# vanilladucky/sde_sampler_lrds

Measured on AMD Instinct MI355X. Metric: particle-steps/sec (batch*n_steps/wall) + log-Z abs-err vs ref, higher is better.
Workload: dtype f32

## Files before the change

sde_sampler_lrds_amd/csrc/prep_kernels.hip:

```cpp
#include "sim_device.hpp"
#include "prep_kernels.hpp"

__global__ void __launch_bounds__(256) k_weight_scales(PackArgs a) {
  __shared__ float red[256];
  float* sc = a.out + sd_off_scales(a.NT);
  {
    const int l = blockIdx.x;
    const float* W = l == 0 ? a.w_in : (l == 1 ? a.w_h1 : (l == 2 ? a.w_h2 : a.w_out));
    const int n = (l == 0 || l == 3) ? SD_H * a.d : SD_H * SD_H;
    float m = 0.0f;
    for (int i = threadIdx.x; i < n; i += 256) {
      const float v = __builtin_fabsf(W[i]);
      m = (v <= 3.0e38f) ? fmaxf(m, v) : m;
    }
    red[threadIdx.x] = m;
    __syncthreads();
    for (int s = 128; s > 0; s >>= 1) {
      if (threadIdx.x < s) red[threadIdx.x] = fmaxf(red[threadIdx.x], red[threadIdx.x + s]);
      __syncthreads();
    }
    if (threadIdx.x == 0) {
      const float mx = red[0];
      int e = 0;
      if (mx > 0.0f && (mx < 9.765625e-4f || mx >= 16384.0f)) {
// ... 78 lines not shown
    float acc = 0.0f;
    for (int i = 0; i < n_in; ++i) acc = __builtin_fmaf(W[i], in[i], acc);
    acc += a.te.b[l][j];
    hbuf[cur][j] = gelu_exact(acc);
    __syncthreads();
    in = hbuf[cur];
    n_in = 64;
    cur ^= 1;
  }
  if (j < a.te.dim_out) {
    const float* W = a.te.w_out + static_cast<size_t>(j) * 64;
    float acc = 0.0f;
    for (int i = 0; i < 64; ++i) acc = __builtin_fmaf(W[i], in[i], acc);
    acc += a.te.b_out[j];
    if (a.clip > 0.0f) acc = clampf(acc, a.clip);
    a.out[static_cast<size_t>(k) * a.te.dim_out + j] = acc;
  }
}

__global__ void __launch_bounds__(128) k_same_var(const float* vars, int K, int d, float* same_var) {
  int differ = 0;
  for (int i = threadIdx.x; i < K * d; i += 128) differ |= vars[i] != vars[i % d];
  differ = __syncthreads_or(differ);
  if (threadIdx.x == 0) same_var[0] = differ ? 0.0f : 1.0f;
}

__global__ void __launch_bounds__(128) k_ref_tables(RefTabArgs a) {
  __shared__ float red[128];
  const int k = blockIdx.x / a.K, c = blockIdx.x % a.K;
  const float S = a.coef[static_cast<size_t>(k) * SDENG_NCOEF + 9];
  const float VA = a.coef[static_cast<size_t>(k) * SDENG_NCOEF + 10];
  const float S2 = a.coef[static_cast<size_t>(k) * SDENG_NCOEF + 11];
  const bool centred = a.centred && a.K == SD_KREG && a.same_var[0] != 0.0f;
  float* tm = a.tab + (static_cast<size_t>(k) * a.K + c) * 2 * a.dpad;
  float* tv = tm + a.dpad;
  float ls = 0.0f, quad = 0.0f;
  for (int f = threadIdx.x; f < a.dpad; f += 128) {
    float mean = 0.0f, iv = 0.0f, cen = 0.0f;
    if (f < a.d) {
      mean = S * a.means[static_cast<size_t>(c) * a.d + f];
      const float var = VA + S2 * a.vars[static_cast<size_t>(c) * a.d + f];
      iv = 1.0f / var;
      ls += logf(var);
      if (centred) {
        float sum = 0.0f;
        for (int j = 0; j < SD_KREG; ++j) sum += a.means[static_cast<size_t>(j) * a.d + f];
        cen = S * (sum * (1.0f / SD_KREG));
      }
    }
    if (centred) {
      const float dm = mean - cen;
      quad = __builtin_fmaf(dm * dm, iv, quad);
      tm[f] = dm * iv;
      tv[f] = c == 0 ? iv : (c == 1 ? cen : 0.0f);
    } else {
      tm[f] = mean;
      tv[f] = iv;
    }
  }
  red[threadIdx.x] = ls;
  __syncthreads();
  for (int s = 64; s > 0; s >>= 1) {
    if (threadIdx.x < s) red[threadIdx.x] += red[threadIdx.x + s];
    __syncthreads();
  }
  const float ls_sum = red[0];
  __syncthreads();
  red[threadIdx.x] = quad;
  __syncthreads();
  for (int s = 64; s > 0; s >>= 1) {
    if (threadIdx.x < s) red[threadIdx.x] += red[threadIdx.x + s];
    __syncthreads();
  }
  if (threadIdx.x == 0) {
    float wsum = 0.0f;
    for (int i = 0; i < a.K; ++i) wsum += a.weights ? a.weights[i] : 1.0f;
    const float w = (a.weights ? a.weights[c] : 1.0f) / wsum;
    float* cs = a.consts + (static_cast<size_t>(k) * a.K + c) * 2;
    cs[0] = 0.5f * ls_sum;
    cs[1] = centred ? logf(w) - 0.5f * red[0] : logf(w);
  }
}

__global__ void __launch_bounds__(256) k_ref_full_tables(RefFullArgs a) {
  __shared__ float invd[128];
  __shared__ float red[256];
  const int k = blockIdx.x / a.K, c = blockIdx.x % a.K;
  const float S = a.coef ? a.coef[static_cast<size_t>(k) * SDENG_NCOEF + 9] : 1.0f;
  const float VA = a.coef ? a.coef[static_cast<size_t>(k) * SDENG_NCOEF + 10] : 0.0f;
  const float S2 = a.coef ? a.coef[static_cast<size_t>(k) * SDENG_NCOEF + 11] : 1.0f;
  const int KB = sd_kb(a.NT);
  const int img_floats = a.NT * KB * 512;
  float ls = 0.0f;
  for (int j = threadIdx.x; j < 128; j += 256) {
    float iv = 0.0f;
    if (j < a.d) {
      const float var = VA + S2 * a.eigvals[static_cast<size_t>(c) * a.d + j];
      iv = 1.0f / var;
      ls += logf(var);
    }
    invd[j] = iv;
  }
  red[threadIdx.x] = ls;
  __syncthreads();
  for (int s = 128; s > 0; s >>= 1) {
    if (threadIdx.x < s) red[threadIdx.x] += red[threadIdx.x + s];
    __syncthreads();
// ... 799 lines not shown
```

sde_sampler_lrds_amd/csrc/prep_kernels.hpp:

```cpp
#pragma once
#include "sim_common.hpp"
#include "../../include/sdeng.h"

#define SD_LOGZ_MAX_BLOCKS 1024

struct PackArgs {
  int NT, d;
  const float *w_in, *b_in, *w_h1, *b_h1, *w_h2, *b_h2, *w_out, *b_out;
  float* out;
  int transpose;
  const float* scales;
};

struct TimeEmbedArgs {
  sdeng_time_embed te;
  const float* coef;
  int col;
  int t_direct;
  float t_value;
  float clip;
  float* out;
};

struct RefTabArgs {
  int K, d, dpad;
  const float* coef;
  const float *means, *vars, *weights;
  float* tab;
  float* consts;
  float* same_var;
  int centred;
};

struct RefFullArgs {
  int K, d, dpad, NT;
  const float* coef;
  const float *means, *eigvals, *eigvecs, *weights;
  float* images;
  float* means_out;
  float* consts;
};

struct RefMMArgs {
  int K, d, dpad, NT, kt;
  const float* coef;
  const float *means, *vars, *weights;
  float* images;
  float* centre;
  float* consts;
  float* same_var;
};

struct DistTabArgs {
  int K, d, dpad;
  const float *loc, *scale, *weights;
  float* tab;
  float* consts;
};

struct DistEvalArgs {
  DistDev ds;
  int B, d, dpad;
  const float* x;
  float* logp_out;
  float* score_out;
};

struct MovesArgs {
  DistEvalArgs prior, target;
  int B, d, K, keep_from, ula;
  float target_acc;
  const float* t;
  float *x, *lp, *grad, *step;
  const float *z, *u;
  unsigned seed_lo, seed_hi;
  long long chain0;
  float* samples;
  float* acc_sum;
  float* acc_last;
};
int sd_launch_moves(const MovesArgs& a, hipStream_t s);

struct TerminalArgs {
  DistDev ref, target;
// ... 18 lines not shown
```

sde_sampler_lrds_amd/csrc/sdeng_api.hip:

```cpp
#include <hip/hip_runtime.h>

#include <algorithm>
#include <cmath>
#include <cstdarg>
#include <cstdio>
#include <cstring>
#include <cstdlib>

#include "../../include/sdeng.h"
#include "prep_kernels.hpp"
#include "sim_kernel.hpp"
#include "cmcd_kernel.hpp"
#include "grad_kernel.hpp"
#include "cmcd_adjoint_kernel.hpp"
#include "metric_kernels.hpp"

int sd_launch_logreg_images(const float* X, const float* y, int n, int dw, int NT, float* image, float* y_pad, hipStream_t s);
int sd_launch_pack_square(const float* P, const float* loc, int d, int NT, float* out, float* loc_pad, hipStream_t s);

static thread_local char g_err[512] = "";
static int fail(int code, const char* fmt, ...) {
  va_list ap;
  va_start(ap, fmt);
  vsnprintf(g_err, sizeof(g_err), fmt, ap);
// ... 500 lines not shown
  SD_TRY(launch_timed(d, p.k, &c, s));
  if (eubo) return terminal(d, dpad, prior, prior, true, false, d->x_out, d->rnd_out, s);
  return terminal(d, dpad, target, target, false, true, d->x_out, d->rnd_out, s);
}

static int run_euler(const SimPlan& p, const sdeng_desc* d, float* ws, SimArgs& a, hipStream_t s) {
  SD_TRY(build_dist(d->target, d->d, 16 * p.DT, ws + p.L.target, a.target, s));
  a.clip_score = d->net.clip_score;
  return launch_timed(d, p.k, &a, s);
}

static int prepare_ref(const SimPlan& p, const sdeng_desc* d, float* ws, SimArgs& a, hipStream_t s) {
  const Layout& L = p.L;
  const int DT = p.DT, dpad = 16 * DT, K = ref_components(d), rf = p.rf;
  if (rf == RF_NONE) return 0;
  a.ref_k = K;
  a.ref_tab = ws + L.ref_tab; a.ref_consts = ws + L.ref_consts;
  a.ref_c1 = half_d_log_2pi(d->d);
  if (rf == RF_GMM_FULL) {
    if (d->N > 0) {
      RefFullArgs r;
      r.K = K; r.d = d->d; r.dpad = dpad; r.NT = DT; r.coef = p.in_slot ? nullptr : d->coef;
      r.means = d->ref.means_init; r.eigvals = d->ref.vars_init; r.eigvecs = d->ref.eigvecs; r.weights = d->ref.weights;
      r.images = ws + L.ref_tab; r.means_out = ws + L.ref_mean; r.consts = ws + L.ref_consts;
      SD_HIP(sd_launch_ref_full_tables(r, d->N, s));
    }
    a.ref_mean = ws + L.ref_mean;
    const int piece = (DT > 4 ? DT / 2 : DT) * sd_kb(DT) * 512;
    a.ref_share = (piece / 256 + SD_WAVES - 1) / SD_WAVES;
    return 0;
  }
  if (rf == RF_GMM_MM) {
    const int kt = (K + 15) / 16;
    if (d->N > 0) {
      RefMMArgs r;
      r.K = K; r.d = d->d; r.dpad = dpad; r.NT = DT; r.kt = kt; r.coef = d->coef;
      r.means = d->ref.means_init; r.vars = d->ref.vars_init; r.weights = d->ref.weights;
      r.images = ws + L.ref_tab; r.centre = ws + L.ref_mean; r.consts = ws + L.ref_consts;
      r.same_var = ws + L.ref_consts + static_cast<size_t>(d->N) * 64;
      SD_HIP(sd_launch_ref_mm_tables(r, d->N, s));
    }
    a.ref_kc = kt;
    a.ref_mean = ws + L.ref_mean;
    a.ref_share = (mm_piece(K, DT) / 256 + SD_WAVES - 1) / SD_WAVES;
    return 0;
  }
  if (d->N > 0) {
    RefTabArgs r;
    r.K = K; r.d = d->d; r.dpad = dpad; r.coef = d->coef;
    r.means = d->ref.means_init; r.vars = d->ref.vars_init; r.weights = rf != RF_GAUSS ? d->ref.weights : nullptr;
    r.tab = ws + L.ref_tab; r.consts = ws + L.ref_consts;
    r.same_var = ws + L.ref_consts + static_cast<size_t>(d->N) * K * 2;
    r.centred = (rf == RF_GMM && p.k.fam != SD_FAM_SPLIT) ? 1 : 0;
    SD_HIP(sd_launch_ref_tables(r, d->N, s));
  }
  a.ref_same_var = ws + L.ref_consts + static_cast<size_t>(d->N) * K * 2;
  if (rf == RF_GMM_BIG) {
    static const bool allow = [] { const char* e = getenv("SDENG_REF_SHARE"); return !(e && e[0] == '0'); }();
    const int cap = std::min(share_room(DT), sd_share_buf_floats(SD_SHARE_MAX)) / 256 * 256;
    const int kc_max = cap / (2 * dpad);
    if (allow && kc_max >= 1) {
      const int nch = (K + kc_max - 1) / kc_max;
      const int kc = (K + nch - 1) / nch;
      const int chunks = (kc * 2 * dpad + 255) / 256;
      a.ref_share = (chunks + SD_WAVES - 1) / SD_WAVES;
      a.ref_kc = kc;
    }
  }
  return 0;
}

static int run_sim(const SimPlan& p, const sdeng_desc* d, float* ws, SimArgs& a, hipStream_t s) {
  const Layout& L = p.L;
  const int DT = p.DT, dpad = 16 * DT;
  SD_TRY(prepare_net(d, L, ws, DT, a, s, d->N, false, 0.0f));
  SD_TRY(prepare_ref(p, d, ws, a, s));
  DistDev target, ref_dist, prior;
  SD_TRY(build_dist(d->target, d->d, dpad, ws + L.target, target, s));
  SD_TRY(build_dist(d->ref_dist, d->d, dpad, ws + L.ref_dist, ref_dist, s));
  SD_TRY(build_dist(d->prior, d->d, dpad, ws + L.prior, prior, s));
  a.target = target;
  a.prior = prior;
  const bool eubo = d->form == SDENG_FORM_EUBO;
  const bool tr = d->flags & SDENG_FLAG_TERM_REF, tt = d->flags & SDENG_FLAG_TERM_TARGET;
  if ((d->flags & SDENG_FLAG_INIT_LOGP) && !eubo) {
    SD_TRY(dist_eval(prior, d->B, d->d, dpad, d->x_in, ws + L.rnd_init, nullptr, s));
    a.rnd_init = ws + L.rnd_init;
  }
  if (eubo && (tr || tt)) {
    SD_HIP(hipMemsetAsync(ws + L.rnd_init, 0, sizeof(float) * d->B, s));
    SD_TRY(terminal(d, dpad, ref_dist, target, tr, tt, d->x_in, ws + L.rnd_init, s));
    a.rnd_init = ws + L.rnd_init;
  }
  if (p.sc == SC_LOGREG) {
    float* unused;
    SD_TRY(prepare_logreg(d, L, ws, DT, a, s, &unused));
  }
  SD_TRY(launch_timed(d, p.k, &a, s));
  if (!eubo && (tr || tt)) SD_TRY(terminal(d, dpad, ref_dist, target, tr, tt, d->x_out, d->rnd_out, s));
  if (eubo && (d->flags & SDENG_FLAG_INIT_LOGP)) SD_TRY(terminal(d, dpad, prior, prior, true, false, d->x_out, d->rnd_out, s));
  return 0;
}

extern "C" int sdeng_simulate(const sdeng_desc* desc, void* stream) {
  hipStream_t s = static_cast<hipStream_t>(stream);
  SimPlan p;
// ... 146 lines not shown
static int check_adjoint(const sdeng_desc* d, bool ext_score) {
  if (!d) return fail(SDENG_E_INVALID, "null descriptor");
  SD_TRY(check_abi(d));
  if (d->d < 1 || d->d > 128 || d->N < 1 || d->B < 1 || !d->coef) return fail(SDENG_E_INVALID, "bad sizes (1 <= d <= 128, N, B >= 1) or null coef");
  if (d->form != SDENG_FORM_LIN && d->form != SDENG_FORM_EM) return fail(SDENG_E_UNSUPPORTED, "kl_adjoint: forward forms LIN / EM (form %d)", d->form);
  if (d->net.ctrl_kind != SDENG_CTRL_CLIPPED &&
      !(score_like(d->net.ctrl_kind) && (ext_score || d->target.kind == SDENG_DIST_GMM_DIAG || d->target.kind == SDENG_DIST_PHI4)))
    return fail(SDENG_E_UNSUPPORTED, "kl_adjoint: ClippedCtrl, or Score / Lerp / CancelDrift control on a diagonal mixture / phi^4 target (ctrl_kind %d, "
                                     "target kind %d)", d->net.ctrl_kind, d->target.kind);
  SD_TRY(check_lerp_prior(d));
  if (d->target.kind == SDENG_DIST_CHECKERBOARD || d->prior.kind == SDENG_DIST_CHECKERBOARD)
    return fail(SDENG_E_UNSUPPORTED, "kl_adjoint: no adjoint for a checkerboard target (KL training takes the per-step path)");
  if (d->ref.kind != SDENG_REF_NONE && d->ref.kind != SDENG_REF_GAUSS_DIAG && d->ref.kind != SDENG_REF_GMM_DIAG)
    return fail(SDENG_E_UNSUPPORTED, "kl_adjoint: no reference, or a diagonal Gaussian / mixture reference (ref.kind %d)", d->ref.kind);
  if (d->ref.kind != SDENG_REF_NONE && ((d->ref.kind == SDENG_REF_GMM_DIAG && d->ref.k < 1) || !d->ref.means_init || !d->ref.vars_init))
    return fail(SDENG_E_INVALID, "reference: null means/vars or k < 1");
  if (static_cast<long long>(d->N) * d->B * d->d >= (1ll << 31)) return fail(SDENG_E_UNSUPPORTED, "N * B * d >= 2^31");
  return check_net(d->net);
}
extern "C" size_t sdeng_kl_adjoint_workspace_bytes(const sdeng_desc* d) {
  if (!d || d->d < 1 || d->d > 128 || d->N < 1) return 0;
  return adjoint_layout(d, tiles_exact(d->d)).total * sizeof(float);
}
extern "C" int sdeng_kl_adjoint(const sdeng_desc* d, const sdeng_adjoint* adj, void* stream) {
  hipStream_t s = static_cast<hipStream_t>(stream);
  SD_TRY(check_adjoint(d, adj && adj->score));
  if (!adj || !adj->xs || !adj->w || !adj->lam_in || !adj->a0 || !adj->a1 || !adj->a2 || !adj->d0 || !adj->d1 || !adj->d2 || !adj->dout)
    return fail(SDENG_E_INVALID, "kl_adjoint: null states / weights / lambda_N / per-row outputs");
  const bool ito = d->flags & SDENG_FLAG_ITO;
  if (ito && !adj->noise) return fail(SDENG_E_INVALID, "kl_adjoint: FLAG_ITO needs the normals of the trajectory");
  const bool score = d->net.ctrl_kind != SDENG_CTRL_CLIPPED;
  if (score && !adj->dst) return fail(SDENG_E_INVALID, "kl_adjoint: a score control needs the dst output");
  if (score && !adj->score) SD_TRY(check_dist(d->target, d->d));
  const int has_score = !score ? ADJ_NONE : adj->score ? ADJ_EXT : (d->target.kind == SDENG_DIST_PHI4 ? ADJ_PHI4 : ADJ_GMM);
  const int DT = tiles_exact(d->d), dpad = 16 * DT;
  KernelKey k;
  SD_TRY(select_kernel(k, SD_FAM_ADJ, DT, has_score));
  const AdjLayout A = adjoint_layout(d, DT);
  const size_t need = A.total * sizeof(float);
  if (!d->workspace || d->workspace_bytes < need) return fail(SDENG_E_WORKSPACE, "workspace %zu bytes, need %zu", d->workspace_bytes, need);
  float* ws = static_cast<float*>(d->workspace);
  AdjArgs a;
  memset(&a, 0, sizeof(a));
  SD_TRY(pack_net(d, DT, ws, ws + A.v.wt, s));
  SD_TRY(embed_times(d, d->N, false, 0.0f, ws + A.v.temb, ws + A.stheta, &a.stheta, s));
  if (d->ref.kind != SDENG_REF_NONE) {
    const int K = ref_components(d);
    RefTabArgs r;
    r.K = K; r.d = d->d; r.dpad = dpad; r.coef = d->coef;
    r.means = d->ref.means_init; r.vars = d->ref.vars_init; r.weights = d->ref.kind == SDENG_REF_GMM_DIAG ? d->ref.weights : nullptr;
    r.tab = ws + A.tab; r.consts = ws + A.consts;
    r.same_var = ws + A.consts + static_cast<size_t>(d->N) * K * 2;
    r.centred = 0;
    SD_HIP(sd_launch_ref_tables(r, d->N, s));
    a.ref_tab = ws + A.tab; a.ref_consts = ws + A.consts; a.ref_k = K;
    a.ref_c1 = half_d_log_2pi(d->d);
  }
  a.has_score = has_score;
  if (score) {
    a.score_ext = adj->score;
    if (!adj->score) SD_TRY(build_dist(d->target, d->d, dpad, ws + A.target, a.target, s));
    a.scale_score = d->net.scale_score; a.clip_score = d->net.clip_score;
    a.ctrl_kind = d->net.ctrl_kind;
    a.prior_loc = d->prior.p0; a.prior_scale = d->net.ctrl_kind == SDENG_CTRL_LERP ? d->prior.p1 : 1.0f;
    a.score_detached = adj->detach_score ? 1 : 0;
    a.dst = adj->dst;
  }
  VjpArgs& v = a.v;
  v.M = d->N * d->B; v.B = d->B; v.d = d->d; v.N = d->N;
  v.x = adj->xs; v.cot = nullptr; v.wpack = ws; v.wpack_t = ws + A.v.wt; v.temb = ws + A.v.temb;
  v.clip_model = d->net.clip_model;
  v.a0 = adj->a0; v.a1 = adj->a1; v.a2 = adj->a2; v.d0 = adj->d0; v.d1 = adj->d1; v.d2 = adj->d2; v.dout = adj->dout;
  v.trash = ws + A.v.trash;
  a.coef = d->coef; a.noise = ito ? adj->noise : nullptr; a.w = adj->w; a.lam_in = adj->lam_in; a.lam_out = adj->lam_out;
  a.lin = d->form == SDENG_FORM_LIN ? 1 : 0;
  a.ntiles_b = (d->B + 15) / 16;
  SD_HIP(k.fn(&a, s));
  return 0;
}

struct CmcdAdjLayout {
  VjpLayout v;
  size_t stheta, target, prior, total;
};
static CmcdAdjLayout cmcd_adjoint_layout(const sdeng_desc* d, int DT) {
  CmcdAdjLayout A;
  A.v = vjp_layout(DT, d->N + 1);
  size_t o = A.v.total;
  A.stheta = o; o += align64(static_cast<size_t>(d->N) + 1);
  A.target = o; o += dist_floats(d->target, 16 * DT);
  A.prior = o; o += dist_floats(d->prior, 16 * DT);
  A.total = o;
  return A;
}
static int check_cmcd_adjoint(const sdeng_desc* d, bool ext_score) {
  if (!d) return fail(SDENG_E_INVALID, "null descriptor");
  SD_TRY(check_abi(d));
  if (d->d > 128) return fail(SDENG_E_UNSUPPORTED, "cmcd_kl_adjoint: d <= 128 (got %d)", d->d);
  if (d->d < 1 || d->N < 1 || d->B < 1 || !d->coef) return fail(SDENG_E_INVALID, "bad sizes (1 <= d, N, B >= 1) or null coef");
  if (d->net.ctrl_kind != SDENG_CTRL_CLIPPED && d->net.ctrl_kind != SDENG_CTRL_SCORE)
    return fail(SDENG_E_UNSUPPORTED, "cmcd_kl_adjoint: ClippedCtrl or ScoreCtrl (ctrl_kind %d)", d->net.ctrl_kind);
  if (d->prior.kind == SDENG_DIST_GAUSS_FULL)
    return fail(SDENG_E_UNSUPPORTED, "cmcd_kl_adjoint: no adjoint for a full-covariance prior (KL training takes the per-step path)");
  if (d->prior.kind != SDENG_DIST_ISO_GAUSS && d->prior.kind != SDENG_DIST_GAUSS_DIAG)
    return fail(SDENG_E_UNSUPPORTED, "cmcd_kl_adjoint: prior must be ISO_GAUSS or GAUSS_DIAG (kind %d)", d->prior.kind);
  switch (d->target.kind) {
// ... 204 lines not shown
```

sde_sampler_lrds_amd/csrc/sim_device.hpp:

```cpp
#pragma once
#include "sim_common.hpp"
#include "../../include/sdeng.h"

#define SD_INLINE __device__ __forceinline__

SD_INLINE float group_sum(float v) {
  v += __shfl_xor(v, 16, 64);
  v += __shfl_xor(v, 32, 64);
  return v;
}
SD_INLINE float exp_nonpos(float v) { return __builtin_amdgcn_exp2f(v * 1.4426950408889634f); }
SD_INLINE float rcp_fast(float v) { return __builtin_amdgcn_rcpf(v); }

SD_INLINE float clampf(float v, float m) {
  v = (v < -m) ? -m : v;
  v = (v > m) ? m : v;
  return v;
}

SD_INLINE void clamp_tile_rare(f32x4& v, float m) {
  bool out_of_range = false;
#pragma unroll
  for (int r = 0; r < 4; ++r) out_of_range |= !(__builtin_fabsf(v[r]) <= m);
  if (__builtin_amdgcn_ballot_w64(out_of_range) != 0) {
// ... 602 lines not shown
#pragma unroll
  for (int r = 0; r < 4; ++r) acc[r] = (acc[r] - x[t][r]) * iv[r];
  return acc;
}

template <int NT>
SD_INLINE void gmm_resp_centred(const f32x4 (&x)[NT], const float* __restrict__ tab, const float* __restrict__ consts, int g,
                                float (&p)[SD_KREG]) {
  constexpr int dpad = 16 * NT;
  float lp[SD_KREG];
#pragma unroll
  for (int k = 0; k < SD_KREG; ++k) lp[k] = 0.0f;
#pragma unroll
  for (int t = 0; t < NT; ++t) {
    const f32x4 y = x[t] - load_tile4(tab + 3 * dpad, t, g);
#pragma unroll
    for (int k = 0; k < SD_KREG; ++k) {
      const f32x4 ak = load_tile4(tab + static_cast<size_t>(k) * 2 * dpad, t, g);
#pragma unroll
      for (int r = 0; r < 4; ++r) lp[k] = __builtin_fmaf(y[r], ak[r], lp[k]);
    }
  }
  float mx = -INFINITY;
#pragma unroll
  for (int k = 0; k < SD_KREG; ++k) {
    lp[k] = consts[2 * k + 1] + group_sum(lp[k]);
    mx = fmaxf(mx, lp[k]);
  }
  float den = 0.0f;
#pragma unroll
  for (int k = 0; k < SD_KREG; ++k) {
    p[k] = exp_nonpos(lp[k] - mx);
    den += p[k];
  }
  const float inv = rcp_fast(den);
#pragma unroll
  for (int k = 0; k < SD_KREG; ++k) p[k] *= inv;
}
template <int NT>
SD_INLINE f32x4 gmm_score_tile_centred(const f32x4 (&x)[NT], const float* __restrict__ tab, int g, const float (&p)[SD_KREG], int t) {
  constexpr int dpad = 16 * NT;
  f32x4 acc = {0.0f, 0.0f, 0.0f, 0.0f};
#pragma unroll
  for (int k = 0; k < SD_KREG; ++k) {
    const f32x4 ak = load_tile4(tab + static_cast<size_t>(k) * 2 * dpad, t, g);
#pragma unroll
    for (int r = 0; r < 4; ++r) acc[r] = __builtin_fmaf(p[k], ak[r], acc[r]);
  }
  const f32x4 iv = load_tile4(tab + dpad, t, g), c = load_tile4(tab + 3 * dpad, t, g);
#pragma unroll
  for (int r = 0; r < 4; ++r) acc[r] = __builtin_fmaf(c[r] - x[t][r], iv[r], acc[r]);
  return acc;
}

template <int NT>
SD_INLINE f32x4 gauss_score_tile(const f32x4 (&x)[NT], const float* __restrict__ tab, int g, int t) {
  constexpr int dpad = 16 * NT;
  const f32x4 m = load_tile4(tab, t, g);
  const f32x4 iv = load_tile4(tab + dpad, t, g);
  f32x4 out;
#pragma unroll
  for (int r = 0; r < 4; ++r) out[r] = -((x[t][r] - m[r]) * iv[r]);
  return out;
}

SD_INLINE f32x4 rings_score(const f32x4& x, const DistDev& ds, int g) {
  const float n = __builtin_sqrtf(x[0] * x[0] + x[1] * x[1]) + 1e-7f;
  const float var = ds.p0 * ds.p0;
  float wsum = 0.0f;
  for (int k = 0; k < ds.k; ++k) wsum += ds.aux1[k];
  const float cn = 0.5f * 1.8378770664093453f + 0.5f * logf(var);
  float lp[8], mx = -INFINITY;
#pragma unroll
  for (int k = 0; k < 8; ++k) {
    lp[k] = -INFINITY;
    if (k < ds.k) {
      const float dl = n - ds.aux0[k];
      lp[k] = logf(ds.aux1[k] / wsum) + ((-0.5f * ((dl * dl) / var)) - cn);
      mx = fmaxf(mx, lp[k]);
    }
  }
  float den = 0.0f, acc = 0.0f;
#pragma unroll
  for (int k = 0; k < 8; ++k) {
    if (k < ds.k) {
      const float e = expf(lp[k] - mx);
      den += e;
      acc += e * ((n - ds.aux0[k]) / var);
    }
  }
  const float sr = -(acc / den);
  const float f = (sr / n) - (1.0f / (n * n));
  return g == 0 ? f32x4{x[0] * f, x[1] * f, 0.0f, 0.0f} : f32x4{0.0f, 0.0f, 0.0f, 0.0f};
}

template <int NT>
SD_INLINE void phi4_edges(const f32x4 (&x)[NT], int t, int g, int lane, float& l_edge, float& r_edge) {
  const int up = (lane + 48) & 63, dn = (lane + 16) & 63;
  const float l_same = __shfl(x[t][3], up, 64);
  const float r_same = __shfl(x[t][0], dn, 64);
  float l_prev = 0.0f, r_next = 0.0f;
  if (t > 0) l_prev = __shfl(x[t > 0 ? t - 1 : 0][3], up, 64);
  if (t < NT - 1) r_next = __shfl(x[t < NT - 1 ? t + 1 : t][0], dn, 64);
  l_edge = (g == 0) ? l_prev : l_same;
  r_edge = (g == 3) ? r_next : r_same;
}
// ... 136 lines not shown
```

sde_sampler_lrds_amd/csrc/sim_kernel.hpp:

```cpp
#pragma once
#include <type_traits>

#include "sim_device.hpp"

enum { RF_NONE = 0, RF_GAUSS = 1, RF_GMM = 2, RF_GMM_BIG = 3, RF_GMM_FULL = 4, RF_GMM_MM = 5 };
enum { SC_NONE = 0, SC_GMM = 1, SC_PHI4 = 2, SC_LOGREG = 3, SC_REFSLOT = 4 };

template <int KIND, bool CLIP>
SD_INLINE float ctrl_score_term(const SimArgs& a, float sv, float xv, float st, float score_gain, float lerp_w, bool in_range,
                                float inv_prior_var) {
  constexpr bool lerp = KIND == SDENG_CTRL_LERP;
  if constexpr (lerp) {
    const float ps = (a.prior.p0 - xv) * inv_prior_var;
    const float df = sv - ps;
    sv = (lerp_w < 0.5f) ? ps + lerp_w * df : sv - df * (1.0f - lerp_w);
  }
  if constexpr (CLIP) sv = clampf(sv, a.clip_score);
  float v = a.scale_score * sv;
  v = v * st;
  if constexpr (lerp) v = in_range ? score_gain * v : 0.0f;
  if constexpr (KIND == SDENG_CTRL_CANCEL_DRIFT) v = in_range ? lerp_w * xv + score_gain * v : 0.0f;
  return v;
}
template <int KIND, bool CLIP>
// ... 78 lines not shown
    if constexpr (SC == SC_LOGREG) {
      const int ni = a.lr.in_lds ? sd_lr_floats(NT, a.lr.n_rows) / 4 : 0;
      for (int i = tid; i < ni; i += THREADS) dst[n4 + i] = reinterpret_cast<const f32x4*>(a.lr.image)[i];
    }
  }
  __syncthreads();
#ifdef SD_STAGGER
  if constexpr (REF != RF_GMM_BIG && REF != RF_GMM_FULL && REF != RF_GMM_MM)
    if (wave >= W / 2)
      for (int i = 0; i < SD_STAGGER; ++i) __builtin_amdgcn_s_sleep(127);
#endif
#ifdef SD_DBG_PRIO_HI47
  if (wave >= 4) __builtin_amdgcn_s_setprio(3);
#endif
#ifdef SD_DBG_ONLY47
  if (wave < 4) return;
#endif
#ifdef SD_DBG_ONLY03
  if (wave >= 4) return;
#endif
  static_assert(SC != SC_LOGREG || (REF == RF_NONE && NT <= 4), "in-loop logistic-regression score: no reference, d <= 64");
  static_assert(SC != SC_REFSLOT || (REF == RF_GMM_FULL && FORM != SDENG_FORM_EUBO), "full-covariance target score: lives in the reference slot, forward forms");
  constexpr bool has_ref = REF != RF_NONE && SC != SC_REFSLOT;
  const float* bias = a.wpack + sd_off_bias(NT);
  const NetScale ns = load_net_scale(bias, NT);
#ifdef SD_NO_RANGE_GUARD
  const bool scaled_net = false;
#else
  const bool scaled_net = ns.any_hidden();
#endif
  const float inv_out_plain = ns.inv_out;
#ifdef SD_DBG_NODMA
  constexpr bool ref_lds = false;
#else
  constexpr bool ref_lds = (REF == RF_GAUSS || REF == RF_GMM);
#endif
  float* my_tab = lds + sd_lds_weight_floats(NT) + wave * SD_REFTAB_FLOATS;
  const int tab_floats = a.ref_k * 2 * dpad;
  const int share = (REF == RF_GMM_BIG || REF == RF_GMM_FULL || REF == RF_GMM_MM) ? __builtin_amdgcn_readfirstlane(a.ref_share) : 0;
  float* sh_tab = lds + sd_lds_weight_floats(NT);
  const int sh_floats = sd_share_buf_floats(share);
  constexpr int FULL_PP = NT > 4 ? 2 : 1, FULL_TO = NT / FULL_PP, FULL_PIECE = FULL_TO * ((NT + 1) / 2) * 512;
  static_assert(REF != RF_GMM_FULL || NT % FULL_PP == 0, "pieces hold whole output tiles");
  const int p = lane & 15, g = lane >> 4;
  constexpr bool lin = FORM == SDENG_FORM_LIN;
  constexpr bool eubo = FORM == SDENG_FORM_EUBO;
  static_assert(!eubo || (SC == SC_NONE) != (REF == RF_NONE), "EUBO kernels: reference-SDE losses with a ClippedCtrl, or DIS (no reference)");
  const bool full_d = a.d == dpad;
  float* trash = a.trash + tid * 4;
  bool same_var = false;
  if constexpr (REF == RF_GMM) same_var = a.N > 0 && a.ref_same_var[0] != 0.0f;
  const bool kfull = REF == RF_GMM && a.ref_k == SD_KREG;
  const bool kfast = kfull && same_var;

  for (int tile = blockIdx.x + gridDim.x * wave; (share ? tile - static_cast<int>(gridDim.x) * wave : tile) < a.ntiles;
       tile += gridDim.x * W) {
    const uint32_t row = static_cast<uint32_t>(tile) * 16u + p;
    const bool live = row < static_cast<uint32_t>(a.B);
    const uint32_t pidx = static_cast<uint32_t>(a.particle0 + row);
    f32x4 x[NT];
    load_rows<NT>(a.x_in, row, a.d, live, g, x);
    float rnd = 0.0f;
    if (a.rnd_init) rnd = (live ? a.rnd_init[row] : 0.0f);
    if constexpr (PAR) {
      if (a.xs_out) store_rows<NT>(a.xs_out, trash, row, a.d, live, g, x);
    }
    if constexpr (ref_lds) {
      if (a.N > 0) dma_table_to_lds(a.ref_tab, my_tab, tab_floats, lane);
    }
    if constexpr (REF == RF_GMM_BIG) {
      if (share) {
        __syncthreads();
        if (a.N > 0) dma_table_shared(a.ref_tab, sh_tab, min(a.ref_kc, a.ref_k) * 2 * dpad, share, wave, lane);
      }
    }
    if constexpr (REF == RF_GMM_MM) {
      __syncthreads();
      if (a.N > 0) dma_table_shared(a.ref_tab, sh_tab, a.ref_kc * ((NT + 1) / 2) * 512, share, wave, lane);
    }
    if constexpr (REF == RF_GMM_FULL) {
      __syncthreads();
      if (a.N > 0) dma_table_shared(a.ref_tab, sh_tab, FULL_PIECE, share, wave, lane);
    }

    for (int k = 0; k < a.N; ++k) {
      const float* cf = a.coef + static_cast<size_t>(k) * SDENG_NCOEF;
      const float c1 = cf[1], c2 = cf[2], c3 = cf[3], c4 = cf[4], c5 = cf[5], c6 = cf[6];
      const float score_gain = cf[7], lerp_w = cf[8];
      const float e1 = __builtin_fmaf(c4, c1, 1.0f), e2 = c4 * c2, e3 = c4 * c3, e4 = c2 * c5;
      int d_dyn = a.d;
      asm volatile("" : "+s"(d_dyn));

      auto noise_tile = [&](int t) -> f32x4 {
        if (PAR && a.noise_in) return load_quad(a.noise_in + static_cast<size_t>(k) * a.B * a.d, row, d_dyn, live, t, g);
        f32x4 z = philox_normal4(pidx, static_cast<uint32_t>(k), static_cast<uint32_t>(4 * t + g), 0u, a.seed_lo, a.seed_hi);
        if constexpr (SC == SC_PHI4) {
          if (!full_d) {
#pragma unroll
            for (int r = 0; r < 4; ++r) z[r] = feat_live<NT>(t, r, 4 * g, d_dyn) ? z[r] : 0.0f;
          }
        }
        return z;
      };
      if constexpr (eubo) {
#pragma unroll
        for (int t = 0; t < NT; ++t) {
          const f32x4 z = noise_tile(t);
#pragma unroll
          for (int r = 0; r < 4; ++r) x[t][r] = x[t][r] * c1 + c3 * z[r];
        }
      }

      f32x4 hid[SD_HT];
      __builtin_amdgcn_s_setprio(2);
      constexpr bool has_twin = REF != RF_GMM_MM && REF != RF_GMM_FULL && SC != SC_LOGREG;
      if constexpr (has_twin) mlp_hidden<NT>(x, hid, lds, bias, a.temb + static_cast<size_t>(k) * SD_H, lane);
      else mlp_hidden_scaled<NT>(x, hid, lds, bias, a.temb + static_cast<size_t>(k) * SD_H, lane, ns);
      __builtin_amdgcn_s_setprio(1);
      HidSplit hs = split_hidden(hid);
      bool safe_net = false;
      float hid_rs = 1.0f;

      f32x4 ts[(SC != SC_NONE && SC != SC_REFSLOT) ? NT : 1];
      if constexpr (SC == SC_GMM) {
        if (NT == 1 && a.target.kind == SDENG_DIST_RINGS) ts[0] = rings_score(x[0], a.target, g);
        else gmm_score<NT>(x, a.target.tab, a.target.consts, 4, a.target.k, a.target.p0, g, ts);
      }
      if constexpr (SC == SC_PHI4) {
        int lane_p = lane;
        if constexpr (NT == 8) asm volatile("" : "+v"(lane_p));
        phi4_score<NT>(x, a.target, d_dyn, g, lane_p, ts);
      }
      if constexpr (SC == SC_LOGREG) {
        asm volatile("" ::: "memory");
        f16x8 xh[(NT + 1) / 2], xl[(NT + 1) / 2];
        split_tiles<NT>(x, xh, xl);
        if (a.lr.in_lds) logreg_score<NT>(x, xh, xl, a.lr, d_dyn, lds + sd_lds_weight_floats(NT), lane, ts);
        else logreg_score<NT>(x, xh, xl, a.lr, d_dyn, a.lr.image, lane, ts);
      }
      const float* rtab = ref_lds ? my_tab : a.ref_tab + static_cast<size_t>(k) * tab_floats;
      const float* rcs = a.ref_consts + static_cast<size_t>(k) * a.ref_k * 2;
      if constexpr (ref_lds) wait_dma();
      float resp[REF == RF_GMM ? SD_KREG : 1];
      f32x4 rs[(REF == RF_GMM_BIG || REF == RF_GMM_FULL || REF == RF_GMM_MM) ? NT : 1];
#ifdef SD_DBG_NOREF
      if constexpr (REF == RF_GMM) { resp[0] = 1.0f; resp[1] = resp[2] = resp[3] = 0.0f; }
#else
      if constexpr (REF == RF_GMM) {
        if (kfast) gmm_resp_centred<NT>(x, rtab, rcs, g, resp);
        else if (kfull) gmm_resp<NT, SD_KREG>(x, rtab, rcs, 2, SD_KREG, a.ref_c1, g, resp);
        else gmm_resp<NT>(x, rtab, rcs, 2, a.ref_k, a.ref_c1, g, resp);
      }
#endif
      if constexpr (REF == RF_GMM_BIG) {
        if (share) {
          const int kc = a.ref_kc, nch = (a.ref_k + kc - 1) / kc;
          float m_run, l_run;
          gmm_score_begin<NT>(rs, m_run, l_run);
          for (int c = 0; c < nch; ++c) {
            const int q = k * nch + c;
            wait_dma();
            __syncthreads();
            const int c2 = c + 1 < nch ? c + 1 : 0, k2 = c + 1 < nch ? k : k + 1;
            if (k2 < a.N)
              dma_table_shared(a.ref_tab + static_cast<size_t>(k2) * tab_floats + c2 * kc * 2 * dpad,
                               sh_tab + ((q + 1) & 1) * sh_floats, min(kc, a.ref_k - c2 * kc) * 2 * dpad, share, wave, lane);
            gmm_score_accum<NT>(x, sh_tab + (q & 1) * sh_floats, rcs + c * kc * 2, 2, min(kc, a.ref_k - c * kc), a.ref_c1, g, rs,
                                m_run, l_run);
          }
          gmm_score_end<NT>(rs, l_run);
        } else {
          gmm_score<NT>(x, rtab, rcs, 2, a.ref_k, a.ref_c1, g, rs);
        }
      }
      if constexpr (REF == RF_GMM_MM) {
        constexpr int KBX = (NT + 1) / 2, KTM = 4;
        const int kt = a.ref_kc, kbk = (kt + 1) / 2;
        const float* cs = a.ref_mean + static_cast<size_t>(k) * 2 * dpad;
        const float* bk = a.ref_consts + static_cast<size_t>(k) * (KTM * 16);
        const int logit_floats = kt * KBX * 512, mean_floats = NT * kbk * 512;
        const float* img = a.ref_tab + static_cast<size_t>(k) * (logit_floats + mean_floats);
        f16x8 ch[KBX], cl[KBX];
        {
          f32x4 xc[NT];
#pragma unroll
          for (int t = 0; t < NT; ++t) xc[t] = x[t] - load_tile4(cs, t, g);
          split_tiles<NT>(xc, ch, cl);
        }
        wait_dma();
        __syncthreads();
        dma_table_shared(img + logit_floats, sh_tab + sh_floats, mean_floats, share, wave, lane);
        f32x4 lt[KTM];
        {
          const f16x8* im = reinterpret_cast<const f16x8*>(sh_tab);
#pragma unroll
          for (int j = 0; j < KTM; ++j) {
            lt[j] = f32x4{-INFINITY, -INFINITY, -INFINITY, -INFINITY};
            if (j < kt) {
              f32x4 acc = load_tile4(bk, j, g), mx = {0.0f, 0.0f, 0.0f, 0.0f};
#pragma unroll
              for (int kb = 0; kb < KBX; ++kb) {
                const f16x8 ah = im[((j * KBX + kb) * 2 + 0) * 64 + lane], al = im[((j * KBX + kb) * 2 + 1) * 64 + lane];
                acc = __builtin_amdgcn_mfma_f32_16x16x32_f16(ah, ch[kb], acc, 0, 0, 0);
// ... 109 lines not shown
      }
      float st = 1.0f;
      if constexpr (SC != SC_NONE) st = a.stheta ? a.stheta[k] : 1.0f;

      float su2 = 0.0f, suz = 0.0f, sux = 0.0f;
      constexpr bool can_remove = SC != SC_NONE && has_ref && !eubo;
      auto ref_tile = [&](int t) __attribute__((always_inline)) -> f32x4 {
        f32x4 rq = {0.0f, 0.0f, 0.0f, 0.0f};
#ifdef SD_DBG_NOREF
        if constexpr (REF == RF_GMM) rq = f32x4{resp[0], resp[0], resp[0], resp[0]};
#else
        if constexpr (REF == RF_GMM) {
          if (kfast) rq = gmm_score_tile_centred<NT>(x, rtab, g, resp, t);
          else if (kfull) rq = gmm_score_tile<NT, SD_KREG>(x, rtab, SD_KREG, g, resp, t);
          else rq = same_var ? gmm_score_tile_shared_var<NT>(x, rtab, a.ref_k, g, resp, t) : gmm_score_tile<NT>(x, rtab, a.ref_k, g, resp, t);
        }
#endif
        if constexpr (REF == RF_GMM_BIG || REF == RF_GMM_FULL || REF == RF_GMM_MM) rq = rs[t];
        if constexpr (REF == RF_GAUSS) rq = gauss_score_tile<NT>(x, rtab, g, t);
        return rq;
      };
      auto out_group = [&](auto otc, int t0) __attribute__((always_inline)) {
        constexpr int OT = decltype(otc)::value;
        f32x4 u[OT];
        if constexpr (has_twin) {
          mlp_out_tiles<NT, OT>(hs, lds, bias, t0, lane, u);
          if (__builtin_expect(safe_net, 0)) out_tiles_unscale<OT>(u, bias, t0, lane, hid_rs, ns.inv_out);
          else if (__builtin_expect(inv_out_plain != 1.0f, 0)) {
            asm volatile("" ::: "memory");
#pragma unroll
            for (int o = 0; o < OT; ++o) u[o] = u[o] * inv_out_plain;
          }
        } else {
          mlp_out_tiles<NT, OT>(hs, lds, bias, t0, lane, u, ns.inv_out);
        }
#ifdef SD_NO_RANGE_GUARD
        constexpr bool range_guard = false;
#else
        constexpr bool range_guard = has_twin;
#endif
        if (has_twin && t0 == 0) {
          const bool bad = range_guard && !(__builtin_fabsf(u[0][0]) <= 3.0e38f);
          const bool trip = scaled_net | (__builtin_amdgcn_ballot_w64(bad) != 0);
          if (__builtin_expect(trip, 0)) {
            asm volatile("" ::: "memory");
            safe_net = true;
            mlp_hidden_safe<NT>(x, hid, lds, bias, a.temb + static_cast<size_t>(k) * SD_H, lane, ns);
            hid_rs = split_hidden_safe(hid, hs);
            mlp_out_tiles<NT, OT>(hs, lds, bias, t0, lane, u);
            out_tiles_unscale<OT>(u, bias, t0, lane, hid_rs, ns.inv_out);
            asm volatile("" ::: "memory");
          }
        }
        if (a.clip_model > 0.0f) {
          bool out_of_range = false;
#pragma unroll
          for (int o = 0; o < OT; ++o)
#pragma unroll
            for (int r = 0; r < 4; ++r) out_of_range |= !(__builtin_fabsf(u[o][r]) <= a.clip_model);
          if (__builtin_amdgcn_ballot_w64(out_of_range) != 0) {
#pragma unroll
            for (int o = 0; o < OT; ++o)
#pragma unroll
              for (int r = 0; r < 4; ++r) u[o][r] = clampf(u[o][r], a.clip_model);
          }
        }
#pragma unroll
        for (int o = 0; o < OT; ++o) {
          const int t = t0 + o;
          if constexpr (SC == SC_REFSLOT) add_ctrl_score_tile(a, u[o], rs[t], x[t], st, score_gain, lerp_w, t, 4 * g, d_dyn);
          else if constexpr (SC != SC_NONE) add_ctrl_score_tile(a, u[o], ts[t], x[t], st, score_gain, lerp_w, t, 4 * g, d_dyn);
          f32x4 rq = {0.0f, 0.0f, 0.0f, 0.0f};
          if constexpr (can_remove) {
            rq = ref_tile(t);
            if (a.flags & SDENG_FLAG_REMOVE_REF) u[o] = u[o] - rq;
          }
          if constexpr (PAR == 2) perturb_ctrl_tile<NT, REF != RF_GMM_FULL>(a, cf, u[o], x[t], pidx, k, t, g, d_dyn);
#pragma unroll
          for (int r = 0; r < 4; ++r) {
            float uv = u[o][r];
            if constexpr (eubo) uv = uv * c2;
            u[o][r] = uv;
            if constexpr (!eubo) su2 = __builtin_fmaf(uv, uv, su2);
          }
          const f32x4 z = noise_tile(t);
          if constexpr (!can_remove && has_ref) rq = ref_tile(t);
#pragma unroll
          for (int r = 0; r < 4; ++r) {
            const float xv = x[t][r], uv = u[o][r];
            if constexpr (eubo) {
              su2 += uv * (rq[r] + 0.5f * uv);
              sux = __builtin_fmaf(uv, xv, sux);
              suz = __builtin_fmaf(uv, z[r], suz);
            } else if constexpr (lin) {
              float sc = uv;
              if constexpr (has_ref) sc = rq[r] + uv;
              x[t][r] = __builtin_fmaf(c3, z[r], __builtin_fmaf(c2, sc, c1 * xv));
              suz = __builtin_fmaf(uv, z[r], suz);
            } else {
              float acc = e1 * xv;
              if constexpr (has_ref) acc = __builtin_fmaf(e3, rq[r], acc);
              x[t][r] = __builtin_fmaf(e4, z[r], __builtin_fmaf(e2, uv, acc));
              suz = __builtin_fmaf(uv, z[r], suz);
            }
          }
        }
      };
#pragma unroll
      for (int t0 = 0; t0 < NT; t0 += 2) {
        if (t0 + 1 < NT) out_group(std::integral_constant<int, 2>{}, t0);
        else out_group(std::integral_constant<int, 1>{}, t0);
      }
      __builtin_amdgcn_s_setprio(0);
      if constexpr (ref_lds) {
        __builtin_amdgcn_sched_barrier(0);
        if (k + 1 < a.N) dma_table_to_lds(a.ref_tab + static_cast<size_t>(k + 1) * tab_floats, my_tab, tab_floats, lane);
      }
      su2 = group_sum(su2);
      if constexpr (eubo) {
        rnd -= su2 * c4;
        if (c6 != 0.0f) rnd += group_sum(sux) * c6;
        rnd -= group_sum(suz) * c5;
      } else {
        rnd += lin ? c4 * su2 : (0.5f * su2) * c4;
        rnd += c6;
        if (a.flags & SDENG_FLAG_ITO) {
          suz = group_sum(suz);
          rnd += c5 * suz;
        }
      }
      if constexpr (PAR) {
        if (a.xs_out) store_rows<NT>(a.xs_out + static_cast<size_t>(k + 1) * a.B * a.d, trash, row, d_dyn, live, g, x);
      }
    }

    store_rows<NT>(a.x_out, trash, row, a.d, live, g, x);
    if (live && g == 0) a.rnd_out[row] = rnd;
  }
// ... 77 lines not shown
```

Measured before the change: 3.361 billion.

## Fuse GMM reference score into state update via precomputed table rows; clip via norm

New measurement: 3.314 billion. -1.4%, worse.

```diff
diff --git a/sde_sampler_lrds_amd/csrc/prep_kernels.hip b/sde_sampler_lrds_amd/csrc/prep_kernels.hip
--- a/sde_sampler_lrds_amd/csrc/prep_kernels.hip
+++ b/sde_sampler_lrds_amd/csrc/prep_kernels.hip
@@ -154,7 +154,15 @@
       const float dm = mean - cen;
       quad = __builtin_fmaf(dm * dm, iv, quad);
       tm[f] = dm * iv;
-      tv[f] = c == 0 ? iv : (c == 1 ? cen : 0.0f);
+      float row = c == 0 ? iv : cen;
+      if (c >= 2) {
+        const float* cf = a.coef + static_cast<size_t>(k) * SDENG_NCOEF;
+        const bool lin = a.form == SDENG_FORM_LIN, em = a.form == SDENG_FORM_EM;
+        const float gx = lin ? cf[1] : __builtin_fmaf(cf[4], cf[1], 1.0f), gr = lin ? cf[2] : cf[4] * cf[3];
+        const double giv = static_cast<double>(gr) * static_cast<double>(iv);
+        row = !(lin || em) ? 0.0f : static_cast<float>(c == 2 ? static_cast<double>(gx) - giv : giv * static_cast<double>(cen));
+      }
+      tv[f] = row;
     } else {
       tm[f] = mean;
       tv[f] = iv;
diff --git a/sde_sampler_lrds_amd/csrc/prep_kernels.hpp b/sde_sampler_lrds_amd/csrc/prep_kernels.hpp
--- a/sde_sampler_lrds_amd/csrc/prep_kernels.hpp
+++ b/sde_sampler_lrds_amd/csrc/prep_kernels.hpp
@@ -30,6 +30,7 @@
   float* consts;
   float* same_var;
   int centred;
+  int form;
 };
 
 struct RefFullArgs {
diff --git a/sde_sampler_lrds_amd/csrc/sdeng_api.hip b/sde_sampler_lrds_amd/csrc/sdeng_api.hip
--- a/sde_sampler_lrds_amd/csrc/sdeng_api.hip
+++ b/sde_sampler_lrds_amd/csrc/sdeng_api.hip
@@ -576,6 +576,7 @@
     r.tab = ws + L.ref_tab; r.consts = ws + L.ref_consts;
     r.same_var = ws + L.ref_consts + static_cast<size_t>(d->N) * K * 2;
     r.centred = (rf == RF_GMM && p.k.fam != SD_FAM_SPLIT) ? 1 : 0;
+    r.form = d->form;
     SD_HIP(sd_launch_ref_tables(r, d->N, s));
   }
   a.ref_same_var = ws + L.ref_consts + static_cast<size_t>(d->N) * K * 2;
@@ -828,6 +829,7 @@
     r.tab = ws + A.tab; r.consts = ws + A.consts;
     r.same_var = ws + A.consts + static_cast<size_t>(d->N) * K * 2;
     r.centred = 0;
+    r.form = d->form;
     SD_HIP(sd_launch_ref_tables(r, d->N, s));
     a.ref_tab = ws + A.tab; a.ref_consts = ws + A.consts; a.ref_k = K;
     a.ref_c1 = half_d_log_2pi(d->d);
diff --git a/sde_sampler_lrds_amd/csrc/sim_device.hpp b/sde_sampler_lrds_amd/csrc/sim_device.hpp
--- a/sde_sampler_lrds_amd/csrc/sim_device.hpp
+++ b/sde_sampler_lrds_amd/csrc/sim_device.hpp
@@ -678,6 +678,21 @@
   for (int r = 0; r < 4; ++r) acc[r] = __builtin_fmaf(c[r] - x[t][r], iv[r], acc[r]);
   return acc;
 }
+template <int NT>
+SD_INLINE void gmm_fused_update_tile(f32x4& xt, const float* __restrict__ tab, int g, const float (&ps)[SD_KREG], int t, const f32x4& u,
+                                     const f32x4& z, float gu, float gz) {
+  constexpr int dpad = 16 * NT;
+  f32x4 acc = load_tile4(tab + 7 * dpad, t, g);
+#pragma unroll
+  for (int k = 0; k < SD_KREG; ++k) {
+    const f32x4 ak = load_tile4(tab + static_cast<size_t>(k) * 2 * dpad, t, g);
+#pragma unroll
+    for (int r = 0; r < 4; ++r) acc[r] = __builtin_fmaf(ps[k], ak[r], acc[r]);
+  }
+  const f32x4 e = load_tile4(tab + 5 * dpad, t, g);
+#pragma unroll
+  for (int r = 0; r < 4; ++r) xt[r] = __builtin_fmaf(gz, z[r], __builtin_fmaf(gu, u[r], __builtin_fmaf(e[r], xt[r], acc[r])));
+}
 
 template <int NT>
 SD_INLINE f32x4 gauss_score_tile(const f32x4 (&x)[NT], const float* __restrict__ tab, int g, int t) {
diff --git a/sde_sampler_lrds_amd/csrc/sim_kernel.hpp b/sde_sampler_lrds_amd/csrc/sim_kernel.hpp
--- a/sde_sampler_lrds_amd/csrc/sim_kernel.hpp
+++ b/sde_sampler_lrds_amd/csrc/sim_kernel.hpp
@@ -154,6 +154,17 @@
   if constexpr (REF == RF_GMM) same_var = a.N > 0 && a.ref_same_var[0] != 0.0f;
   const bool kfull = REF == RF_GMM && a.ref_k == SD_KREG;
   const bool kfast = kfull && same_var;
+#if defined(SD_NO_FUSED_UPDATE) || defined(SD_DBG_NOREF)
+  constexpr bool can_fuse = false;
+#else
+  constexpr bool can_fuse = REF == RF_GMM && SC == SC_NONE && !eubo && PAR != 2;
+#endif
+#ifdef SD_NO_COST_CLIP
+  constexpr bool cost_clip = false;
+#else
+  constexpr bool cost_clip = SC == SC_NONE && !eubo && PAR != 2 && REF != RF_GMM_MM && REF != RF_GMM_FULL;
+#endif
+  const float clip_sq = a.clip_model * a.clip_model;
 
   for (int tile = blockIdx.x + gridDim.x * wave; (share ? tile - static_cast<int>(gridDim.x) * wave : tile) < a.ntiles;
        tile += gridDim.x * W) {
@@ -249,8 +260,14 @@
       if constexpr (REF == RF_GMM) { resp[0] = 1.0f; resp[1] = resp[2] = resp[3] = 0.0f; }
 #else
       if constexpr (REF == RF_GMM) {
-        if (kfast) gmm_resp_centred<NT>(x, rtab, rcs, g, resp);
-        else if (kfull) gmm_resp<NT, SD_KREG>(x, rtab, rcs, 2, SD_KREG, a.ref_c1, g, resp);
+        if (kfast) {
+          gmm_resp_centred<NT>(x, rtab, rcs, g, resp);
+          if constexpr (can_fuse) {
+            const float gr = lin ? c2 : e3;
+#pragma unroll
+            for (int kc = 0; kc < SD_KREG; ++kc) resp[kc] *= gr;
+          }
+        } else if (kfull) gmm_resp<NT, SD_KREG>(x, rtab, rcs, 2, SD_KREG, a.ref_c1, g, resp);
         else gmm_resp<NT>(x, rtab, rcs, 2, a.ref_k, a.ref_c1, g, resp);
       }
 #endif
@@ -466,7 +483,25 @@
             asm volatile("" ::: "memory");
           }
         }
-        if (a.clip_model > 0.0f) {
+        if constexpr (cost_clip) {
+          const float su2_in = su2;
+#pragma unroll
+          for (int o = 0; o < OT; ++o)
+#pragma unroll
+            for (int r = 0; r < 4; ++r) su2 = __builtin_fmaf(u[o][r], u[o][r], su2);
+          if (a.clip_model > 0.0f) {
+            if (__builtin_expect(__builtin_amdgcn_ballot_w64(!(su2 < clip_sq)) != 0, 0)) {
+              su2 = su2_in;
+#pragma unroll
+              for (int o = 0; o < OT; ++o)
+#pragma unroll
+                for (int r = 0; r < 4; ++r) {
+                  u[o][r] = clampf(u[o][r], a.clip_model);
+                  su2 = __builtin_fmaf(u[o][r], u[o][r], su2);
+                }
+            }
+          }
+        } else if (a.clip_model > 0.0f) {
           bool out_of_range = false;
 #pragma unroll
           for (int o = 0; o < OT; ++o)
@@ -495,9 +530,17 @@
             float uv = u[o][r];
             if constexpr (eubo) uv = uv * c2;
             u[o][r] = uv;
-            if constexpr (!eubo) su2 = __builtin_fmaf(uv, uv, su2);
+            if constexpr (!eubo && !cost_clip) su2 = __builtin_fmaf(uv, uv, su2);
           }
           const f32x4 z = noise_tile(t);
+          if constexpr (can_fuse) {
+            if (kfast) {
+              gmm_fused_update_tile<NT>(x[t], rtab, g, resp, t, u[o], z, lin ? c2 : e2, lin ? c3 : e4);
+#pragma unroll
+              for (int r = 0; r < 4; ++r) suz = __builtin_fmaf(u[o][r], z[r], suz);
+              continue;
+            }
+          }
           if constexpr (!can_remove && has_ref) rq = ref_tile(t);
 #pragma unroll
           for (int r = 0; r < 4; ++r) {
```
